# zzbuzzard/PATHS

Measured on AMD Instinct MI355X. Metric: slides_per_sec_5level_K2048_D1024, higher is better.
Workload: dtype f32 (products as 2 fp16 planes per operand = 22 bits, 3 fp16 MFMAs per block, fp32 accumulate); 1 GPU; 5-level PATHS recursion (forward, eval): K=2048 patches/level (level-0 grid 32x64, top_k 512, 10% background), D=1024 features, trans_dim 128 x 4 heads x 2 layers, LSTM ctx 256; 8 HBM-resident slides per GPU; slides_per_gpu=8, global_batch=8, levels=5, resident_batches_rotated=3, parallelism=slide-sharded x1 (no data-path collective)

## Files before the change

### paths_amd/csrc/token0_ws.hip

```cpp
#include "common.h"
#include "lanes.h"

namespace {

constexpr int DM = 128, DFF = 512, NH = 4, HD = 32;
constexpr int NT = 512;
constexpr int SLOTS = NT / 32;
constexpr int REC = 4 + DM;
constexpr int MAX_TS = 16;
constexpr int TS_TOKENS = 128;

constexpr int OFF_A = 0;
constexpr int OFF_A0 = OFF_A + NH * DM * DM;
constexpr int OFF_WV = OFF_A0 + NH * DM;
constexpr int OFF_WO = OFF_WV + DM * DM;
constexpr int OFF_W1 = OFF_WO + DM * DM;
constexpr int OFF_W2 = OFF_W1 + DFF * DM;
constexpr int OFF_OB = OFF_W2 + DM * DFF;
constexpr int IMG_FLOATS = OFF_OB + DM;


struct T0Params {
  const float* x1;
  const int64_t* num_ims;
  const float* img;
  const float *bv, *bo, *ln1g, *ln1b, *cab, *ln2g, *ln2b, *b1, *b2, *ln3g, *ln3b, *lnfg, *lnfb;
  const float* ctx_prev; int64_t ctx_stride; const float* ctx_all; int ctx_depth;
  const float* wcls; const float* bcls; int num_logits, cls_in;
  float* ctx_out; float* logits;
  float* partials;
  int* counters;
  int* status;
  int T, nts; float eps, eps_f;
  int special_last;
};

__device__ __forceinline__ void st_agent(float* p, float v) { __hip_atomic_store(p, v, __ATOMIC_RELAXED, __HIP_MEMORY_SCOPE_AGENT); }
__device__ __forceinline__ float ld_agent(const float* p) { return __hip_atomic_load(p, __ATOMIC_RELAXED, __HIP_MEMORY_SCOPE_AGENT); }
__device__ __forceinline__ float dot4(f32x4 a, f32x4 b) { return fmaf(a[3], b[3], fmaf(a[2], b[2], fmaf(a[1], b[1], a[0] * b[0]))); }

__device__ __forceinline__ void block_layernorm(float* v, const float* g, const float* bta, float eps, int tid) {
  if (tid < 64) {
    const float a = v[tid], c = v[tid + 64];
    const float mean = wave_sum64(a + c) * (1.0f / DM);
    const float da = a - mean, dc = c - mean;
    const float rstd = 1.0f / sqrtf(wave_sum64(da * da + dc * dc) * (1.0f / DM) + eps);
    v[tid] = da * rstd * g[tid] + bta[tid];
    v[tid + 64] = dc * rstd * g[tid + 64] + bta[tid + 64];
  }
  __syncthreads();
}

__global__ void __launch_bounds__(NT)
token0_ws_kernel(T0Params p) {
  __shared__ __attribute__((aligned(16))) float smem[SLOTS * DM + 4 * DFF + 8 * DM + 64];
  float* const sZ = smem;
  float* const sRed = smem + SLOTS * DM;
  float* const sV = sRed + 4 * DFF;
  float* const sX0 = sV, *const sQ = sV + DM, *const sO = sV + 2 * DM, *const sXa = sV + 3 * DM, *const sY = sV + 4 * DM;
  float* const sML = sV + 5 * DM;
  int* const sFlag = reinterpret_cast<int*>(sV + 5 * DM + 2 * SLOTS);
  const int b = blockIdx.y, head = blockIdx.x & 3, ts = blockIdx.x >> 2;
  const int tid = threadIdx.x, lane = tid & 63, wave = tid >> 6;
  const float* xb = p.x1 + (int64_t)b * p.T * DM;

  if (tid < DM) sX0[tid] = xb[(p.special_last ? (int64_t)min((int)p.num_ims[b], p.T - 1) * DM : 0) + tid];
  __syncthreads();
  {
    const int c = tid & 127, kq = tid >> 7;
    const float* A = p.img + OFF_A + (int64_t)head * DM * DM;
    f32x4 w[8];
#pragma unroll
    for (int i = 0; i < 8; ++i) w[i] = ldg_f32x4(A + ((8 * kq + i) * DM + c) * 4);
    float acc = 0.f;
#pragma unroll
    for (int i = 0; i < 8; ++i) acc += dot4(w[i], *reinterpret_cast<const f32x4*>(sX0 + 32 * kq + 4 * i));
    sRed[kq * DM + c] = acc;
  }
  __syncthreads();
  if (tid < DM) sQ[tid] = ((sRed[tid] + sRed[DM + tid]) + (sRed[2 * DM + tid] + sRed[3 * DM + tid])) + p.img[OFF_A0 + head * DM + tid];
  __syncthreads();

  const int len = min((int)p.num_ims[b] + 1, p.T);
  const int chunk = (len + p.nts - 1) / p.nts;
  const int k0 = ts * chunk, k1 = min(len, k0 + chunk);
  const int l5 = lane & 31, slot = wave * 2 + (lane >> 5);
  const f32x4 qv = *reinterpret_cast<const f32x4*>(sQ + 4 * l5);
  float m = -1e30f, l = 0.f;
  f32x4 z = {0.f, 0.f, 0.f, 0.f};
  for (int base = k0; base < k1; base += 8 * SLOTS) {
    f32x4 x[8];
    float s[8];
    bool ok[8];
#pragma unroll
    for (int u = 0; u < 8; ++u) {
      const int tok = base + u * SLOTS + slot;
      ok[u] = tok < k1;
      x[u] = ldg_f32x4(xb + (int64_t)min(tok, k1 - 1) * DM + 4 * l5);
    }
    float mx = m;
#pragma unroll
    for (int u = 0; u < 8; ++u) {
      s[u] = ok[u] ? half_sum32(dot4(qv, x[u])) : -1e30f;
      mx = fmaxf(mx, s[u]);
    }
    const float alpha = __builtin_amdgcn_exp2f(m - mx);
    float ps = 0.f;
    z = z * alpha;
#pragma unroll
    for (int u = 0; u < 8; ++u) {
      const float pu = ok[u] ? __builtin_amdgcn_exp2f(s[u] - mx) : 0.f;
      ps += pu;
      z = z + x[u] * pu;
    }
    l = l * alpha + ps;
    m = mx;
  }
  *reinterpret_cast<f32x4*>(sZ + slot * DM + 4 * l5) = z;
  if (l5 == 0) { sML[2 * slot] = m; sML[2 * slot + 1] = l; }
  __syncthreads();
  float* rec = p.partials + (((int64_t)b * NH + head) * p.nts + ts) * REC;
  if (tid < DM) {
    float M = -1e30f;
#pragma unroll
    for (int sl = 0; sl < SLOTS; ++sl) M = fmaxf(M, sML[2 * sl]);
    float num = 0.f, den = 0.f;
#pragma unroll
    for (int sl = 0; sl < SLOTS; ++sl) {
      const float w = __builtin_amdgcn_exp2f(sML[2 * sl] - M);
      num = fmaf(sZ[sl * DM + tid], w, num);
      den = fmaf(sML[2 * sl + 1], w, den);
    }
    st_agent(rec + 4 + tid, num);
    if (tid == 0) { st_agent(rec, M); st_agent(rec + 1, den); }
  }
  asm volatile("s_waitcnt vmcnt(0)" ::: "memory");
  __syncthreads();
  if (tid == 0) {
    const int total = NH * p.nts;
    const int t = __hip_atomic_fetch_add(p.counters + 3 * b, 1, __ATOMIC_ACQ_REL, __HIP_MEMORY_SCOPE_AGENT);
    const int last = (t == total - 1) ? 1 : 0;
    if (last) {
      __builtin_amdgcn_fence(__ATOMIC_ACQUIRE, "agent");
      __hip_atomic_store(p.counters + 3 * b, 0, __ATOMIC_RELAXED, __HIP_MEMORY_SCOPE_AGENT);
    }
    *sFlag = last;
  }
  __syncthreads();
  if (*sFlag == 0) return;

  const float* W = p.img;
  const int f = tid & 127, kq = tid >> 7;
  float pm[MAX_TS], pl[MAX_TS], pz[MAX_TS];
  {
    const float* hp = p.partials + ((int64_t)b * NH + kq) * p.nts * REC;
#pragma unroll
    for (int t = 0; t < MAX_TS; ++t) {
      const int tc = min(t, p.nts - 1);
      pm[t] = ld_agent(hp + tc * REC); pl[t] = ld_agent(hp + tc * REC + 1); pz[t] = ld_agent(hp + tc * REC + 4 + f);
    }
  }
  f32x4 wv[8], wo[8], w1[32];
#pragma unroll
  for (int i = 0; i < 8; ++i) wv[i] = ldg_f32x4(W + OFF_WV + ((8 * kq + i) * DM + f) * 4);
#pragma unroll
  for (int i = 0; i < 8; ++i) wo[i] = ldg_f32x4(W + OFF_WO + ((8 * kq + i) * DM + f) * 4);
#pragma unroll
  for (int i = 0; i < 32; ++i) w1[i] = ldg_f32x4(W + OFF_W1 + (i * DFF + tid) * 4);
  {
    float M = -1e30f;
#pragma unroll
    for (int t = 0; t < MAX_TS; ++t) if (t < p.nts) M = fmaxf(M, pm[t]);
    float num = 0.f, den = 0.f;
#pragma unroll
    for (int t = 0; t < MAX_TS; ++t)
      if (t < p.nts) {
        const float w = __builtin_amdgcn_exp2f(pm[t] - M);
        num = fmaf(pz[t], w, num);
        den = fmaf(pl[t], w, den);
      }
    sZ[kq * DM + f] = num / den;
  }
  __syncthreads();
  {
    const float* zc = sZ + (f >> 5) * DM + 32 * kq;
    float acc = 0.f;
#pragma unroll
    for (int i = 0; i < 8; ++i) acc += dot4(wv[i], *reinterpret_cast<const f32x4*>(zc + 4 * i));
    sRed[kq * DM + f] = acc;
  }
  __syncthreads();
  if (tid < DM) sO[tid] = ((sRed[tid] + sRed[DM + tid]) + (sRed[2 * DM + tid] + sRed[3 * DM + tid])) + p.bv[tid];
  __syncthreads();
  f32x4 w2[32];
#pragma unroll
  for (int i = 0; i < 16; ++i) w2[i] = ldg_f32x4(W + OFF_W2 + ((32 * kq + i) * DM + f) * 4);
  {
    float acc = 0.f;
#pragma unroll
    for (int i = 0; i < 8; ++i) acc += dot4(wo[i], *reinterpret_cast<const f32x4*>(sO + 32 * kq + 4 * i));
    sRed[kq * DM + f] = acc;
  }
  __syncthreads();
  if (tid < DM) sXa[tid] = sX0[tid] + (((sRed[tid] + sRed[DM + tid]) + (sRed[2 * DM + tid] + sRed[3 * DM + tid])) + p.bo[tid]);
  __syncthreads();
  block_layernorm(sXa, p.ln1g, p.ln1b, p.eps, tid);
  if (tid < DM) sXa[tid] += p.cab[tid];
  __syncthreads();
  block_layernorm(sXa, p.ln2g, p.ln2b, p.eps, tid);
  {
    float acc = 0.f;
#pragma unroll
    for (int i = 0; i < 32; ++i) acc += dot4(w1[i], *reinterpret_cast<const f32x4*>(sXa + 4 * i));
    sRed[tid] = fmaxf(acc + p.b1[tid], 0.f);
  }
#pragma unroll
  for (int i = 16; i < 32; ++i) w2[i] = ldg_f32x4(W + OFF_W2 + ((32 * kq + i) * DM + f) * 4);
  __syncthreads();
  {
    float acc = 0.f;
#pragma unroll
    for (int i = 0; i < 32; ++i) acc += dot4(w2[i], *reinterpret_cast<const f32x4*>(sRed + 128 * kq + 4 * i));
    sZ[kq * DM + f] = acc;
  }
  __syncthreads();
  if (tid < DM) sXa[tid] = sXa[tid] + (((sZ[tid] + sZ[DM + tid]) + (sZ[2 * DM + tid] + sZ[3 * DM + tid])) + p.b2[tid]);
  __syncthreads();
  block_layernorm(sXa, p.ln3g, p.ln3b, p.eps, tid);
  block_layernorm(sXa, p.lnfg, p.lnfb, p.eps_f, tid);
  if (tid < DM) {
    float v = sXa[tid];
    if (p.ctx_prev) v += p.ctx_prev[(int64_t)b * p.ctx_stride + tid];
    sXa[tid] = v;
    p.ctx_out[(int64_t)b * DM + tid] = v;
  }
  __syncthreads();
  for (int j = wave; j < p.num_logits; j += NT / 64) {
    const float* w = p.wcls + (int64_t)j * p.cls_in;
    float acc = 0.f;
    if (p.ctx_all) {
      for (int i = lane; i < p.ctx_depth * DM; i += 64) acc += w[i] * p.ctx_all[(int64_t)b * p.ctx_depth * DM + i];
      w += p.ctx_depth * DM;
    }
    acc += w[lane] * sXa[lane] + w[lane + 64] * sXa[lane + 64];
    acc = wave_sum64(acc);
    if (lane == 0) p.logits[(int64_t)b * p.num_logits + j] = acc + p.bcls[j];
  }
}


constexpr int SPIN_LIMIT = 1 << 22;

template <int D_>
struct T0G {
  static_assert(D_ % 64 == 0 && D_ >= 128 && D_ <= 256, "token0 distributed form: trans_dim 128 or 192 (256 untested)");
  static constexpr int DM = D_, DFF = 4 * D_, HD = D_ / NH, NT = 4 * D_, SLOTS = NT / 32, FPL = D_ / 32, REC = 4 + D_;
  static constexpr int NV = D_ / 64;
  static constexpr int NQ = D_ / 16;
  static constexpr int MAXLD = D_ == 128 ? 8 : D_ / 32;
  static constexpr int RT = D_ == 128 ? 8 : 4;
  static constexpr int OFF_A = 0;
  static constexpr int OFF_A0 = OFF_A + NH * DM * DM;
  static constexpr int OFF_WV = OFF_A0 + NH * DM;
  static constexpr int OFF_WO = OFF_WV + DM * DM;
  static constexpr int OFF_W1 = OFF_WO + DM * DM;
  static constexpr int OFF_W2 = OFF_W1 + DFF * DM;
  static constexpr int OFF_OB = OFF_W2 + DM * DFF;
  static constexpr int IMG_FLOATS = OFF_OB + DM;
  static constexpr int SMEM = SLOTS * DM + 4 * DFF + 8 * DM + 64;
};
static_assert(T0G<128>::OFF_OB == OFF_OB && T0G<128>::IMG_FLOATS == IMG_FLOATS && T0G<128>::REC == REC && T0G<128>::NT == NT, "one image layout at 128");

template <int FPL>
__device__ __forceinline__ void ld_feats(const float* p, float (&x)[FPL]) {
  if constexpr (FPL == 4) {
    const f32x4 t = ldg_f32x4(p);
    x[0] = t[0]; x[1] = t[1]; x[2] = t[2]; x[3] = t[3];
  } else {
    static_assert(FPL % 2 == 0, "features per lane");
    typedef const f32x2 __attribute__((address_space(1))) * gptr;
#pragma unroll
    for (int i = 0; i < FPL / 2; ++i) {
      const f32x2 t = *reinterpret_cast<gptr>(reinterpret_cast<uintptr_t>(p + 2 * i));
      x[2 * i] = t[0]; x[2 * i + 1] = t[1];
    }
  }
}
template <int FPL>
__device__ __forceinline__ float dot_feats(const float (&a)[FPL], const float (&b)[FPL]) {
  float acc = a[0] * b[0];
#pragma unroll
  for (int i = 1; i < FPL; ++i) acc = fmaf(a[i], b[i], acc);
  return acc;
}
template <int D>
__device__ __forceinline__ void block_layernorm_d(float* v, const float* g, const float* bta, float eps, int tid) {
  if (tid < 64) {
    constexpr int VP = D / 64;
    float a[VP], s = 0.f;
#pragma unroll
    for (int i = 0; i < VP; ++i) { a[i] = v[tid + 64 * i]; s += a[i]; }
    const float mean = wave_sum64(s) * (1.0f / D);
    float q = 0.f;
#pragma unroll
    for (int i = 0; i < VP; ++i) { a[i] -= mean; q = fmaf(a[i], a[i], q); }
    const float rstd = 1.0f / sqrtf(wave_sum64(q) * (1.0f / D) + eps);
#pragma unroll
    for (int i = 0; i < VP; ++i) v[tid + 64 * i] = a[i] * rstd * g[tid + 64 * i] + bta[tid + 64 * i];
  }
  __syncthreads();
}

template <int D_>
__global__ void __launch_bounds__(4 * D_)
token0_dist_kernel(T0Params p) {
  using G_ = T0G<D_>;
  constexpr int DM = G_::DM, DFF = G_::DFF, HD = G_::HD, NT = G_::NT, SLOTS = G_::SLOTS, FPL = G_::FPL, REC = G_::REC;
  constexpr int NV = G_::NV, NQ = G_::NQ, MAXLD = G_::MAXLD, RT = G_::RT;
  constexpr int OFF_A = G_::OFF_A, OFF_A0 = G_::OFF_A0, OFF_WV = G_::OFF_WV, OFF_WO = G_::OFF_WO, OFF_W1 = G_::OFF_W1, OFF_W2 = G_::OFF_W2, OFF_OB = G_::OFF_OB;
  __shared__ __attribute__((aligned(16))) float smem[G_::SMEM];
  float* const sZ = smem;
  float* const sRed = smem + SLOTS * DM;
  float* const sV = sRed + 4 * DFF;
  float* const sX0 = sV, *const sQ = sV + DM, *const sNum = sV + 2 * DM, *const sXa = sV + 3 * DM, *const sH = sV + 4 * DM;
  float* const sML = sV + 5 * DM;
  float* const sVv = sV + 5 * DM + 2 * SLOTS + 8;
  int* const sFlag = reinterpret_cast<int*>(sV + 5 * DM + 2 * SLOTS);
  const int G = NH * p.nts, HS = DFF / G, nld = HS / 16;
  const int b = blockIdx.y, j = blockIdx.x, head = j & 3, ts = j >> 2;
  const int tid = threadIdx.x, lane = tid & 63, wave = tid >> 6;
  const float* xb = p.x1 + (int64_t)b * p.T * DM;
  const float* W = p.img;

  const int o5 = tid % HD, kq5 = tid / HD;
  const int f7 = tid % DM, kq7 = tid / DM;
  const int n1 = tid % HS, kq1 = tid / HS;
  f32x4 wv[NV], wo[NV], w1[MAXLD], w2[MAXLD];
#pragma unroll
  for (int i = 0; i < NV; ++i) {
    wv[i] = ldg_f32x4(W + OFF_WV + ((NV * kq5 + i) * DM + HD * head + o5) * 4);
    wo[i] = ldg_f32x4(W + OFF_WO + (((HD / 4) * head + NV * kq7 + i) * DM + f7) * 4);
  }
#pragma unroll
  for (int i = 0; i < MAXLD; ++i)
    if (i < nld) {
      w1[i] = ldg_f32x4(W + OFF_W1 + ((kq1 * nld + i) * DFF + j * HS + n1) * 4);
      w2[i] = ldg_f32x4(W + OFF_W2 + (((j * HS) / 4 + kq7 * nld + i) * DM + f7) * 4);
    }

  constexpr bool A_EARLY = DM == 128;
  const float* const A = W + OFF_A + (int64_t)head * DM * DM;
  f32x4 w[NQ];
  if constexpr (A_EARLY) {
#pragma unroll
    for (int i = 0; i < NQ; ++i) w[i] = ldg_f32x4(A + ((NQ * kq7 + i) * DM + f7) * 4);
  }
  const int len = min((int)p.num_ims[b] + 1, p.T);
  const int chunk = (len + p.nts - 1) / p.nts;
  const int k0 = ts * chunk, k1 = min(len, k0 + chunk);
  const int l5 = lane & 31, slot = wave * 2 + (lane >> 5);
  float xa[RT][FPL], xn[RT][FPL];
  auto fetch = [&](float (&dst)[RT][FPL], int base) __attribute__((always_inline)) {
#pragma unroll
    for (int u = 0; u < RT; ++u) ld_feats<FPL>(xb + (int64_t)max(min(base + u * SLOTS + slot, k1 - 1), 0) * DM + FPL * l5, dst[u]);
  };
  if (A_EARLY && k0 < k1) fetch(xa, k0);

  if (tid < DM) sX0[tid] = xb[(p.special_last ? (int64_t)min((int)p.num_ims[b], p.T - 1) * DM : 0) + tid];
  __syncthreads();
  {
    if constexpr (!A_EARLY) {
#pragma unroll
      for (int i = 0; i < NQ; ++i) w[i] = ldg_f32x4(A + ((NQ * kq7 + i) * DM + f7) * 4);
    }
    float acc = 0.f;
#pragma unroll
    for (int i = 0; i < NQ; ++i) acc += dot4(w[i], *reinterpret_cast<const f32x4*>(sX0 + (DM / 4) * kq7 + 4 * i));
    sRed[kq7 * DM + f7] = acc;
  }
  __syncthreads();
  if (tid < DM) sQ[tid] = ((sRed[tid] + sRed[DM + tid]) + (sRed[2 * DM + tid] + sRed[3 * DM + tid])) + W[OFF_A0 + head * DM + tid];
// ... 44 lines not shown
  if (l5 == 0) { sML[2 * slot] = m; sML[2 * slot + 1] = l; }
  __syncthreads();
  float Mloc = -1e30f;
#pragma unroll
  for (int sl = 0; sl < SLOTS; ++sl) Mloc = fmaxf(Mloc, sML[2 * sl]);
  if (tid < DM) {
    float num = 0.f;
#pragma unroll
    for (int sl = 0; sl < SLOTS; ++sl) num = fmaf(sZ[sl * DM + tid], __builtin_amdgcn_exp2f(sML[2 * sl] - Mloc), num);
    sNum[tid] = num;
  }
  float den = 0.f;
#pragma unroll
  for (int sl = 0; sl < SLOTS; ++sl) den = fmaf(sML[2 * sl + 1], __builtin_amdgcn_exp2f(sML[2 * sl] - Mloc), den);
  __syncthreads();
  {
    float acc = 0.f;
#pragma unroll
    for (int i = 0; i < NV; ++i) acc += dot4(wv[i], *reinterpret_cast<const f32x4*>(sNum + 4 * (NV * kq5 + i)));
    sRed[kq5 * HD + o5] = acc;
  }
  __syncthreads();
  if (tid < HD) {
    float acc = 0.f;
#pragma unroll
    for (int k = 0; k < NT / HD; ++k) acc += sRed[k * HD + tid];
    sVv[tid] = acc;
  }
  __syncthreads();
  {
    float acc = 0.f;
#pragma unroll
    for (int i = 0; i < NV; ++i) acc += dot4(wo[i], *reinterpret_cast<const f32x4*>(sVv + 4 * (NV * kq7 + i)));
    sRed[2 * DFF + kq7 * DM + f7] = acc;
  }
  __syncthreads();
  float* rec = p.partials + ((int64_t)b * G + j) * REC;
  if (tid < DM) {
    const float* r4 = sRed + 2 * DFF + tid;
    st_agent(rec + 4 + tid, (r4[0] + r4[DM]) + (r4[2 * DM] + r4[3 * DM]));
    if (tid == 0) { st_agent(rec, Mloc); st_agent(rec + 1, den); }
  }
  asm volatile("s_waitcnt vmcnt(0)" ::: "memory");
  __syncthreads();
  int* cnt = p.counters + 3 * b;
  if (tid == 0) {
    __hip_atomic_fetch_add(cnt, 1, __ATOMIC_RELEASE, __HIP_MEMORY_SCOPE_AGENT);
    int spins = 0;
    while (__hip_atomic_load(cnt, __ATOMIC_RELAXED, __HIP_MEMORY_SCOPE_AGENT) < G) {
      __builtin_amdgcn_s_sleep(1);
      if (++spins > SPIN_LIMIT) {
        if (p.status) atomicOr(p.status, 4);
        break;
      }
    }
    __builtin_amdgcn_fence(__ATOMIC_ACQUIRE, "agent");
  }
  __syncthreads();
  {
    const int h = kq7;
    const float* hp = p.partials + (int64_t)b * G * REC;
    float pm[8], pl[8], pu[8];
#pragma unroll
    for (int t = 0; t < 8; ++t) {
      const int tc = min(t, p.nts - 1);
      const float* r = hp + (tc * NH + h) * REC;
      pm[t] = ld_agent(r); pl[t] = ld_agent(r + 1); pu[t] = ld_agent(r + 4 + f7);
    }
    float M = -1e30f;
#pragma unroll
    for (int t = 0; t < 8; ++t) if (t < p.nts) M = fmaxf(M, pm[t]);
    float num = 0.f, dn = 0.f;
#pragma unroll
    for (int t = 0; t < 8; ++t)
      if (t < p.nts) {
        const float w = __builtin_amdgcn_exp2f(pm[t] - M);
        num = fmaf(pu[t], w, num);
        dn = fmaf(pl[t], w, dn);
      }
    sRed[h * DM + f7] = num / dn;
  }
  __syncthreads();
  if (tid < DM) sXa[tid] = sX0[tid] + (((sRed[tid] + sRed[DM + tid]) + (sRed[2 * DM + tid] + sRed[3 * DM + tid])) + W[OFF_OB + tid]);
  __syncthreads();
  block_layernorm_d<DM>(sXa, p.ln1g, p.ln1b, p.eps, tid);
  if (tid < DM) sXa[tid] += p.cab[tid];
  __syncthreads();
  block_layernorm_d<DM>(sXa, p.ln2g, p.ln2b, p.eps, tid);
  {
    float acc = 0.f;
#pragma unroll
    for (int i = 0; i < MAXLD; ++i)
      if (i < nld) acc += dot4(w1[i], *reinterpret_cast<const f32x4*>(sXa + (kq1 * nld + i) * 4));
    sRed[kq1 * HS + n1] = acc;
  }
  __syncthreads();
  if (tid < HS) {
    float acc = 0.f;
    const int ng = NT / HS;
    for (int k = 0; k < ng; ++k) acc += sRed[k * HS + tid];
    sH[tid] = fmaxf(acc + p.b1[j * HS + tid], 0.f);
  }
  __syncthreads();
  {
    float acc = 0.f;
#pragma unroll
    for (int i = 0; i < MAXLD; ++i)
      if (i < nld) acc += dot4(w2[i], *reinterpret_cast<const f32x4*>(sH + (kq7 * nld + i) * 4));
    sRed[2 * DFF + kq7 * DM + f7] = acc;
  }
  __syncthreads();
  float* rec2 = p.partials + (int64_t)gridDim.y * (G * REC + DM) + ((int64_t)b * G + j) * DM;
  if (tid < DM) {
    const float* r4 = sRed + 2 * DFF + tid;
    st_agent(rec2 + tid, (r4[0] + r4[DM]) + (r4[2 * DM] + r4[3 * DM]));
  }
  asm volatile("s_waitcnt vmcnt(0)" ::: "memory");
  __syncthreads();
  if (tid == 0) *sFlag = (__hip_atomic_fetch_add(cnt + 2, 1, __ATOMIC_ACQ_REL, __HIP_MEMORY_SCOPE_AGENT) == G - 1) ? 1 : 0;
  __syncthreads();
  if (*sFlag == 0) return;
  if (tid == 0) {
    __hip_atomic_store(cnt, 0, __ATOMIC_RELAXED, __HIP_MEMORY_SCOPE_AGENT);
    __hip_atomic_store(cnt + 2, 0, __ATOMIC_RELAXED, __HIP_MEMORY_SCOPE_AGENT);
  }
  {
    const float* r2 = p.partials + (int64_t)gridDim.y * (G * REC + DM) + (int64_t)b * G * DM;
    float acc = 0.f;
    for (int g = kq7; g < G; g += 4) acc += ld_agent(r2 + g * DM + f7);
    sRed[kq7 * DM + f7] = acc;
  }
  __syncthreads();
  if (tid < DM) sXa[tid] = sXa[tid] + (((sRed[tid] + sRed[DM + tid]) + (sRed[2 * DM + tid] + sRed[3 * DM + tid])) + p.b2[tid]);
  __syncthreads();
  block_layernorm_d<DM>(sXa, p.ln3g, p.ln3b, p.eps, tid);
  block_layernorm_d<DM>(sXa, p.lnfg, p.lnfb, p.eps_f, tid);
  if (tid < DM) {
    float v = sXa[tid];
    if (p.ctx_prev) v += p.ctx_prev[(int64_t)b * p.ctx_stride + tid];
    sXa[tid] = v;
    p.ctx_out[(int64_t)b * DM + tid] = v;
  }
  __syncthreads();
  for (int jj = wave; jj < p.num_logits; jj += NT / 64) {
    const float* w = p.wcls + (int64_t)jj * p.cls_in;
    float acc = 0.f;
    if (p.ctx_all) {
      for (int i = lane; i < p.ctx_depth * DM; i += 64) acc += w[i] * p.ctx_all[(int64_t)b * p.ctx_depth * DM + i];
      w += p.ctx_depth * DM;
    }
#pragma unroll
    for (int i = 0; i < DM / 64; ++i) acc += w[lane + 64 * i] * sXa[lane + 64 * i];
    acc = wave_sum64(acc);
    if (lane == 0) p.logits[(int64_t)b * p.num_logits + jj] = acc + p.bcls[jj];
  }
}

template <int D_>
__global__ void __launch_bounds__(256)
token0_pack_kernel(const float* __restrict__ wqkv, const float* __restrict__ bqkv, const float* __restrict__ wo, const float* __restrict__ bo,
                   const float* __restrict__ w1, const float* __restrict__ w2, float qscale, float* __restrict__ out) {
  using G_ = T0G<D_>;
// ... 4 lines not shown
    if (i >= NH * DM * DM) return;
    const int e = i & 3, c = (i >> 2) % DM, r_ = (i >> 2) / DM, k4 = r_ % (DM / 4), h = r_ / (DM / 4);
    const float* wq = wqkv + (int64_t)(HD * h) * DM + 4 * k4 + e;
    const float* wk = wqkv + (int64_t)(DM + HD * h) * DM + c;
    float acc = 0.f;
    for (int r = 0; r < HD; ++r) acc = fmaf(wk[r * DM], wq[r * DM], acc);
    out[G_::OFF_A + i] = acc * qscale;
  } else if (job == 1) {
    if (i >= NH * DM) return;
    const int c = i % DM, h = i / DM;
    const float* wk = wqkv + (int64_t)(DM + HD * h) * DM + c;
    float acc = 0.f;
    for (int r = 0; r < HD; ++r) acc = fmaf(wk[r * DM], bqkv[HD * h + r], acc);
    out[G_::OFF_A0 + i] = acc * qscale;
  } else if (job == 6) {
    if (i >= DM) return;
    float acc = 0.f;
    for (int k = 0; k < DM; ++k) acc = fmaf(wo[(int64_t)i * DM + k], bqkv[2 * DM + k], acc);
    out[G_::OFF_OB + i] = acc + bo[i];
  } else {
    const float* src; int N, K, off;
    if (job == 2) { src = wqkv + 2 * DM * DM; N = DM; K = DM; off = G_::OFF_WV; }
    else if (job == 3) { src = wo; N = DM; K = DM; off = G_::OFF_WO; }
    else if (job == 4) { src = w1; N = DFF; K = DM; off = G_::OFF_W1; }
    else { src = w2; N = DM; K = DFF; off = G_::OFF_W2; }
    if (i >= N * K) return;
    const int e = i & 3, n = (i >> 2) % N, k4 = (i >> 2) / N;
    out[off + i] = src[(int64_t)n * K + 4 * k4 + e];
  }
}

}

template <int D_>
static int dist_limit() {
  static int cached[64] = {0};
  int dev = 0;
  if (hipGetDevice(&dev) != hipSuccess || dev < 0 || dev >= 64) return 0;
  if (cached[dev] == 0) {
    int cus = 0, occ = 0;
    if (hipDeviceGetAttribute(&cus, hipDeviceAttributeMultiprocessorCount, dev) != hipSuccess || cus <= 0) return 0;
    if (hipOccupancyMaxActiveBlocksPerMultiprocessor(&occ, reinterpret_cast<const void*>(token0_dist_kernel<D_>), T0G<D_>::NT, 0) != hipSuccess || occ <= 0) return 0;
    cached[dev] = cus * (occ > 1 ? 1 : occ) * 3 / 4;
  }
  return cached[dev];
}
static int dist_splits(int B, int T, int d) {
  const int limit = d == 192 ? dist_limit<192>() : dist_limit<128>();
  for (int nts = d == 192 ? 4 : 8; nts >= (d == 192 ? 2 : 1); nts >>= 1)
    if (NH * nts * B <= limit && (nts == 1 || (nts - 1) * TS_TOKENS < T)) return nts;
  return 0;
}
static int chain_splits(int T) {
  int nts = (T + TS_TOKENS - 1) / TS_TOKENS;
  return nts < 1 ? 1 : nts > MAX_TS ? MAX_TS : nts;
}

extern "C" {

int64_t paths_token0_ws_image_bytes_d(int d) { return d == 192 ? (int64_t)T0G<192>::IMG_FLOATS * 4 : d == 128 ? (int64_t)IMG_FLOATS * 4 : 0; }
int64_t paths_token0_ws_image_bytes(void) { return paths_token0_ws_image_bytes_d(128); }

int paths_token0_ws_supported(int B, int T, int d, int H) {
  if (H != NH || B <= 0 || T <= 0) return 0;
  if (d == 128) return 1;
  if (d == 192) return dist_splits(B, T, d) > 0 ? 1 : 0;
  return 0;
}

int64_t paths_token0_ws_partials_d(int B, int T, int d) {
  const int rec = 4 + d;
  const int64_t chain = d == 128 ? (int64_t)B * NH * chain_splits(T) * rec : 0;
  const int nd = dist_splits(B, T, d);
  const int64_t dist = nd ? (int64_t)B * (NH * nd * (rec + d) + d) : 0;
  return chain > dist ? chain : dist;
}
int64_t paths_token0_ws_partials(int B, int T) { return paths_token0_ws_partials_d(B, T, 128); }

int paths_token0_pack_ws_d(const float* wqkv, const float* bqkv, const float* wo, const float* bo, const float* w1, const float* w2, float qscale,
                           int d, void* out, hipStream_t stream) {
  PATHS_REQUIRE(wqkv && bqkv && wo && bo && w1 && w2 && out && (uintptr_t)out % 16 == 0, "token0_pack_ws: bad arguments");
  PATHS_REQUIRE(d == 128 || d == 192, "token0_pack_ws: trans_dim must be 128 or 192 (got %d)", d);
  const dim3 grid((unsigned)(4 * d * d / 256), 7);
  if (d == 192) hipLaunchKernelGGL(token0_pack_kernel<192>, grid, dim3(256), 0, stream, wqkv, bqkv, wo, bo, w1, w2, qscale, reinterpret_cast<float*>(out));
  else hipLaunchKernelGGL(token0_pack_kernel<128>, grid, dim3(256), 0, stream, wqkv, bqkv, wo, bo, w1, w2, qscale, reinterpret_cast<float*>(out));
  PATHS_LAUNCH_CHECK("token0_pack_ws");
  return PATHS_OK;
}
int paths_token0_pack_ws(const float* wqkv, const float* bqkv, const float* wo, const float* bo, const float* w1, const float* w2, float qscale,
                         void* out, hipStream_t stream) {
  return paths_token0_pack_ws_d(wqkv, bqkv, wo, bo, w1, w2, qscale, 128, out, stream);
}

int paths_token0_tail_ws(const float* x1, const int64_t* num_ims, const void* img, const float* bv, const float* bo,
                         const float* ln1g, const float* ln1b, const float* cab, const float* ln2g, const float* ln2b,
                         const float* b1, const float* b2, const float* ln3g, const float* ln3b, const float* lnfg, const float* lnfb,
                         const float* ctx_prev, int64_t ctx_stride, const float* ctx_all, int ctx_depth,
                         const float* wcls, const float* bcls, int num_logits, int cls_in,
                         float* ctx_out, float* logits, float* partials, int* counters, int* status, int B, int T, int d, int H,
                         float eps, float eps_final, int special_last, hipStream_t stream) {
  PATHS_REQUIRE((d == 128 || d == 192) && H == NH, "token0_tail_ws: this build supports trans_dim 128 or 192 with 4 heads (got %d, %d)", d, H);
  PATHS_REQUIRE(B > 0 && T > 0 && x1 && num_ims && img && bv && bo && ln1g && ln1b && cab && ln2g && ln2b && b1 && b2 && ln3g && ln3b && lnfg && lnfb,
                "token0_tail_ws: null operand");
  PATHS_REQUIRE(wcls && bcls && ctx_out && logits && partials && counters, "token0_tail_ws: null output / scratch");
  PATHS_REQUIRE(num_logits > 0 && cls_in == (ctx_all ? (ctx_depth + 1) * d : d), "token0_tail_ws: bad classifier shape");
  PATHS_REQUIRE(((uintptr_t)x1 | (uintptr_t)img) % 16 == 0, "token0_tail_ws: buffers must be 16-byte aligned");
  const int nd = dist_splits(B, T, d);
  if (d != 128 && nd == 0)
    return paths_set_error(PATHS_EUNSUPPORTED, "token0_tail_ws: trans_dim %d has the distributed form only and %d slides do not fit it (paths_token0_ws_supported)", d, B);
  const int nts = nd ? nd : chain_splits(T);
  T0Params p{x1, num_ims, reinterpret_cast<const float*>(img), bv, bo, ln1g, ln1b, cab, ln2g, ln2b, b1, b2, ln3g, ln3b, lnfg, lnfb,
             ctx_prev, ctx_stride, ctx_all, ctx_depth, wcls, bcls, num_logits, cls_in, ctx_out, logits, partials, counters, status, T, nts, eps, eps_final, special_last ? 1 : 0};
  if (nd && d == 192) hipLaunchKernelGGL(token0_dist_kernel<192>, dim3(NH * nts, B), dim3(T0G<192>::NT), 0, stream, p);
  else if (nd) hipLaunchKernelGGL(token0_dist_kernel<128>, dim3(NH * nts, B), dim3(NT), 0, stream, p);
  else hipLaunchKernelGGL(token0_ws_kernel, dim3(NH * nts, B), dim3(NT), 0, stream, p);
  PATHS_LAUNCH_CHECK("token0_tail_ws");
  return PATHS_OK;
}

}
```

Baseline: 3754 slides/s.

## Split token0 tail into pass and chain kernels, replacing grid-wide spin barrier

The distributed token0 kernel used a spin-wait barrier across all attention blocks of a slide before running the feed-forward slices, and a separate chain kernel served other cases. This replaces both with two launches. A pass kernel computes per-head, per-split attention partials. A chain kernel then merges them and computes the FFN across a fixed 8 workgroups per slide, with a last-block reduction. Removing the spin barrier and the occupancy-based split selection avoids co-residency requirements and idle spinning, at the cost of an extra kernel launch and a round trip of the partials through global memory. MAX_TS is lowered to 4.

```diff
diff --git a/paths_amd/csrc/token0_ws.hip b/paths_amd/csrc/token0_ws.hip
--- a/paths_amd/csrc/token0_ws.hip
+++ b/paths_amd/csrc/token0_ws.hip
@@ -3,34 +3,21 @@
 
 namespace {
 
-constexpr int DM = 128, DFF = 512, NH = 4, HD = 32;
-constexpr int NT = 512;
-constexpr int SLOTS = NT / 32;
-constexpr int REC = 4 + DM;
-constexpr int MAX_TS = 16;
+constexpr int NH = 4;
+constexpr int MAX_TS = 4;
 constexpr int TS_TOKENS = 128;
-
-constexpr int OFF_A = 0;
-constexpr int OFF_A0 = OFF_A + NH * DM * DM;
-constexpr int OFF_WV = OFF_A0 + NH * DM;
-constexpr int OFF_WO = OFF_WV + DM * DM;
-constexpr int OFF_W1 = OFF_WO + DM * DM;
-constexpr int OFF_W2 = OFF_W1 + DFF * DM;
-constexpr int OFF_OB = OFF_W2 + DM * DFF;
-constexpr int IMG_FLOATS = OFF_OB + DM;
-
+constexpr int G2 = 8;
 
 struct T0Params {
   const float* x1;
   const int64_t* num_ims;
   const float* img;
-  const float *bv, *bo, *ln1g, *ln1b, *cab, *ln2g, *ln2b, *b1, *b2, *ln3g, *ln3b, *lnfg, *lnfb;
+  const float *ln1g, *ln1b, *cab, *ln2g, *ln2b, *b1, *b2, *ln3g, *ln3b, *lnfg, *lnfb;
   const float* ctx_prev; int64_t ctx_stride; const float* ctx_all; int ctx_depth;
   const float* wcls; const float* bcls; int num_logits, cls_in;
   float* ctx_out; float* logits;
   float* partials;
   int* counters;
-  int* status;
   int T, nts; float eps, eps_f;
   int special_last;
 };
@@ -39,225 +26,15 @@
 __device__ __forceinline__ float ld_agent(const float* p) { return __hip_atomic_load(p, __ATOMIC_RELAXED, __HIP_MEMORY_SCOPE_AGENT); }
 __device__ __forceinline__ float dot4(f32x4 a, f32x4 b) { return fmaf(a[3], b[3], fmaf(a[2], b[2], fmaf(a[1], b[1], a[0] * b[0]))); }
 
-__device__ __forceinline__ void block_layernorm(float* v, const float* g, const float* bta, float eps, int tid) {
-  if (tid < 64) {
-    const float a = v[tid], c = v[tid + 64];
-    const float mean = wave_sum64(a + c) * (1.0f / DM);
-    const float da = a - mean, dc = c - mean;
-    const float rstd = 1.0f / sqrtf(wave_sum64(da * da + dc * dc) * (1.0f / DM) + eps);
-    v[tid] = da * rstd * g[tid] + bta[tid];
-    v[tid + 64] = dc * rstd * g[tid + 64] + bta[tid + 64];
-  }
-  __syncthreads();
-}
-
-__global__ void __launch_bounds__(NT)
-token0_ws_kernel(T0Params p) {
-  __shared__ __attribute__((aligned(16))) float smem[SLOTS * DM + 4 * DFF + 8 * DM + 64];
-  float* const sZ = smem;
-  float* const sRed = smem + SLOTS * DM;
-  float* const sV = sRed + 4 * DFF;
-  float* const sX0 = sV, *const sQ = sV + DM, *const sO = sV + 2 * DM, *const sXa = sV + 3 * DM, *const sY = sV + 4 * DM;
-  float* const sML = sV + 5 * DM;
-  int* const sFlag = reinterpret_cast<int*>(sV + 5 * DM + 2 * SLOTS);
-  const int b = blockIdx.y, head = blockIdx.x & 3, ts = blockIdx.x >> 2;
-  const int tid = threadIdx.x, lane = tid & 63, wave = tid >> 6;
-  const float* xb = p.x1 + (int64_t)b * p.T * DM;
-
-  if (tid < DM) sX0[tid] = xb[(p.special_last ? (int64_t)min((int)p.num_ims[b], p.T - 1) * DM : 0) + tid];
-  __syncthreads();
-  {
-    const int c = tid & 127, kq = tid >> 7;
-    const float* A = p.img + OFF_A + (int64_t)head * DM * DM;
-    f32x4 w[8];
-#pragma unroll
-    for (int i = 0; i < 8; ++i) w[i] = ldg_f32x4(A + ((8 * kq + i) * DM + c) * 4);
-    float acc = 0.f;
-#pragma unroll
-    for (int i = 0; i < 8; ++i) acc += dot4(w[i], *reinterpret_cast<const f32x4*>(sX0 + 32 * kq + 4 * i));
-    sRed[kq * DM + c] = acc;
-  }
-  __syncthreads();
-  if (tid < DM) sQ[tid] = ((sRed[tid] + sRed[DM + tid]) + (sRed[2 * DM + tid] + sRed[3 * DM + tid])) + p.img[OFF_A0 + head * DM + tid];
-  __syncthreads();
-
-  const int len = min((int)p.num_ims[b] + 1, p.T);
-  const int chunk = (len + p.nts - 1) / p.nts;
-  const int k0 = ts * chunk, k1 = min(len, k0 + chunk);
-  const int l5 = lane & 31, slot = wave * 2 + (lane >> 5);
-  const f32x4 qv = *reinterpret_cast<const f32x4*>(sQ + 4 * l5);
-  float m = -1e30f, l = 0.f;
-  f32x4 z = {0.f, 0.f, 0.f, 0.f};
-  for (int base = k0; base < k1; base += 8 * SLOTS) {
-    f32x4 x[8];
-    float s[8];
-    bool ok[8];
-#pragma unroll
-    for (int u = 0; u < 8; ++u) {
-      const int tok = base + u * SLOTS + slot;
-      ok[u] = tok < k1;
-      x[u] = ldg_f32x4(xb + (int64_t)min(tok, k1 - 1) * DM + 4 * l5);
-    }
-    float mx = m;
-#pragma unroll
-    for (int u = 0; u < 8; ++u) {
-      s[u] = ok[u] ? half_sum32(dot4(qv, x[u])) : -1e30f;
-      mx = fmaxf(mx, s[u]);
-    }
-    const float alpha = __builtin_amdgcn_exp2f(m - mx);
-    float ps = 0.f;
-    z = z * alpha;
-#pragma unroll
-    for (int u = 0; u < 8; ++u) {
-      const float pu = ok[u] ? __builtin_amdgcn_exp2f(s[u] - mx) : 0.f;
-      ps += pu;
-      z = z + x[u] * pu;
-    }
-    l = l * alpha + ps;
-    m = mx;
-  }
-  *reinterpret_cast<f32x4*>(sZ + slot * DM + 4 * l5) = z;
-  if (l5 == 0) { sML[2 * slot] = m; sML[2 * slot + 1] = l; }
-  __syncthreads();
-  float* rec = p.partials + (((int64_t)b * NH + head) * p.nts + ts) * REC;
-  if (tid < DM) {
-    float M = -1e30f;
-#pragma unroll
-    for (int sl = 0; sl < SLOTS; ++sl) M = fmaxf(M, sML[2 * sl]);
-    float num = 0.f, den = 0.f;
-#pragma unroll
-    for (int sl = 0; sl < SLOTS; ++sl) {
-      const float w = __builtin_amdgcn_exp2f(sML[2 * sl] - M);
-      num = fmaf(sZ[sl * DM + tid], w, num);
-      den = fmaf(sML[2 * sl + 1], w, den);
-    }
-    st_agent(rec + 4 + tid, num);
-    if (tid == 0) { st_agent(rec, M); st_agent(rec + 1, den); }
-  }
-  asm volatile("s_waitcnt vmcnt(0)" ::: "memory");
-  __syncthreads();
-  if (tid == 0) {
-    const int total = NH * p.nts;
-    const int t = __hip_atomic_fetch_add(p.counters + 3 * b, 1, __ATOMIC_ACQ_REL, __HIP_MEMORY_SCOPE_AGENT);
-    const int last = (t == total - 1) ? 1 : 0;
-    if (last) {
-      __builtin_amdgcn_fence(__ATOMIC_ACQUIRE, "agent");
-      __hip_atomic_store(p.counters + 3 * b, 0, __ATOMIC_RELAXED, __HIP_MEMORY_SCOPE_AGENT);
-    }
-    *sFlag = last;
-  }
-  __syncthreads();
-  if (*sFlag == 0) return;
-
-  const float* W = p.img;
-  const int f = tid & 127, kq = tid >> 7;
-  float pm[MAX_TS], pl[MAX_TS], pz[MAX_TS];
-  {
-    const float* hp = p.partials + ((int64_t)b * NH + kq) * p.nts * REC;
-#pragma unroll
-    for (int t = 0; t < MAX_TS; ++t) {
-      const int tc = min(t, p.nts - 1);
-      pm[t] = ld_agent(hp + tc * REC); pl[t] = ld_agent(hp + tc * REC + 1); pz[t] = ld_agent(hp + tc * REC + 4 + f);
-    }
-  }
-  f32x4 wv[8], wo[8], w1[32];
-#pragma unroll
-  for (int i = 0; i < 8; ++i) wv[i] = ldg_f32x4(W + OFF_WV + ((8 * kq + i) * DM + f) * 4);
-#pragma unroll
-  for (int i = 0; i < 8; ++i) wo[i] = ldg_f32x4(W + OFF_WO + ((8 * kq + i) * DM + f) * 4);
-#pragma unroll
-  for (int i = 0; i < 32; ++i) w1[i] = ldg_f32x4(W + OFF_W1 + (i * DFF + tid) * 4);
-  {
-    float M = -1e30f;
-#pragma unroll
-    for (int t = 0; t < MAX_TS; ++t) if (t < p.nts) M = fmaxf(M, pm[t]);
-    float num = 0.f, den = 0.f;
-#pragma unroll
-    for (int t = 0; t < MAX_TS; ++t)
-      if (t < p.nts) {
-        const float w = __builtin_amdgcn_exp2f(pm[t] - M);
-        num = fmaf(pz[t], w, num);
-        den = fmaf(pl[t], w, den);
-      }
-    sZ[kq * DM + f] = num / den;
-  }
-  __syncthreads();
-  {
-    const float* zc = sZ + (f >> 5) * DM + 32 * kq;
-    float acc = 0.f;
-#pragma unroll
-    for (int i = 0; i < 8; ++i) acc += dot4(wv[i], *reinterpret_cast<const f32x4*>(zc + 4 * i));
-    sRed[kq * DM + f] = acc;
-  }
-  __syncthreads();
-  if (tid < DM) sO[tid] = ((sRed[tid] + sRed[DM + tid]) + (sRed[2 * DM + tid] + sRed[3 * DM + tid])) + p.bv[tid];
-  __syncthreads();
-  f32x4 w2[32];
-#pragma unroll
-  for (int i = 0; i < 16; ++i) w2[i] = ldg_f32x4(W + OFF_W2 + ((32 * kq + i) * DM + f) * 4);
-  {
-    float acc = 0.f;
-#pragma unroll
-    for (int i = 0; i < 8; ++i) acc += dot4(wo[i], *reinterpret_cast<const f32x4*>(sO + 32 * kq + 4 * i));
-    sRed[kq * DM + f] = acc;
-  }
-  __syncthreads();
-  if (tid < DM) sXa[tid] = sX0[tid] + (((sRed[tid] + sRed[DM + tid]) + (sRed[2 * DM + tid] + sRed[3 * DM + tid])) + p.bo[tid]);
-  __syncthreads();
-  block_layernorm(sXa, p.ln1g, p.ln1b, p.eps, tid);
-  if (tid < DM) sXa[tid] += p.cab[tid];
-  __syncthreads();
-  block_layernorm(sXa, p.ln2g, p.ln2b, p.eps, tid);
-  {
-    float acc = 0.f;
-#pragma unroll
-    for (int i = 0; i < 32; ++i) acc += dot4(w1[i], *reinterpret_cast<const f32x4*>(sXa + 4 * i));
-    sRed[tid] = fmaxf(acc + p.b1[tid], 0.f);
-  }
-#pragma unroll
-  for (int i = 16; i < 32; ++i) w2[i] = ldg_f32x4(W + OFF_W2 + ((32 * kq + i) * DM + f) * 4);
-  __syncthreads();
-  {
-    float acc = 0.f;
-#pragma unroll
-    for (int i = 0; i < 32; ++i) acc += dot4(w2[i], *reinterpret_cast<const f32x4*>(sRed + 128 * kq + 4 * i));
-    sZ[kq * DM + f] = acc;
-  }
-  __syncthreads();
-  if (tid < DM) sXa[tid] = sXa[tid] + (((sZ[tid] + sZ[DM + tid]) + (sZ[2 * DM + tid] + sZ[3 * DM + tid])) + p.b2[tid]);
-  __syncthreads();
-  block_layernorm(sXa, p.ln3g, p.ln3b, p.eps, tid);
-  block_layernorm(sXa, p.lnfg, p.lnfb, p.eps_f, tid);
-  if (tid < DM) {
-    float v = sXa[tid];
-    if (p.ctx_prev) v += p.ctx_prev[(int64_t)b * p.ctx_stride + tid];
-    sXa[tid] = v;
-    p.ctx_out[(int64_t)b * DM + tid] = v;
-  }
-  __syncthreads();
-  for (int j = wave; j < p.num_logits; j += NT / 64) {
-    const float* w = p.wcls + (int64_t)j * p.cls_in;
-    float acc = 0.f;
-    if (p.ctx_all) {
-      for (int i = lane; i < p.ctx_depth * DM; i += 64) acc += w[i] * p.ctx_all[(int64_t)b * p.ctx_depth * DM + i];
-      w += p.ctx_depth * DM;
-    }
-    acc += w[lane] * sXa[lane] + w[lane + 64] * sXa[lane + 64];
-    acc = wave_sum64(acc);
-    if (lane == 0) p.logits[(int64_t)b * p.num_logits + j] = acc + p.bcls[j];
-  }
-}
-
-
-constexpr int SPIN_LIMIT = 1 << 22;
-
 template <int D_>
 struct T0G {
-  static_assert(D_ % 64 == 0 && D_ >= 128 && D_ <= 256, "token0 distributed form: trans_dim 128 or 192 (256 untested)");
+  static_assert(D_ % 64 == 0 && D_ >= 128 && D_ <= 256, "token0 tail: trans_dim 128 or 192 (256 untested)");
   static constexpr int DM = D_, DFF = 4 * D_, HD = D_ / NH, NT = 4 * D_, SLOTS = NT / 32, FPL = D_ / 32, REC = 4 + D_;
   static constexpr int NV = D_ / 64;
   static constexpr int NQ = D_ / 16;
-  static constexpr int MAXLD = D_ == 128 ? 8 : D_ / 32;
+  static constexpr int HS = 4 * D_ / G2;
+  static constexpr int NLD = HS / 16;
+  static_assert(HS % 16 == 0 && (4 * D_) % HS == 0 && HS <= D_, "feed-forward slice: a multiple of 16 hidden units that divides the workgroup");
   static constexpr int RT = D_ == 128 ? 8 : 4;
   static constexpr int OFF_A = 0;
   static constexpr int OFF_A0 = OFF_A + NH * DM * DM;
@@ -267,9 +44,9 @@
   static constexpr int OFF_W2 = OFF_W1 + DFF * DM;
   static constexpr int OFF_OB = OFF_W2 + DM * DFF;
   static constexpr int IMG_FLOATS = OFF_OB + DM;
-  static constexpr int SMEM = SLOTS * DM + 4 * DFF + 8 * DM + 64;
+  static constexpr int SMEM_PASS = SLOTS * DM + 8 * DM + 4 * DM + 2 * SLOTS + 8 + HD;
+  static constexpr int SMEM_CHAIN = 8 * DM + 3 * DM + 8;
 };
-static_assert(T0G<128>::OFF_OB == OFF_OB && T0G<128>::IMG_FLOATS == IMG_FLOATS && T0G<128>::REC == REC && T0G<128>::NT == NT, "one image layout at 128");
 
 template <int FPL>
 __device__ __forceinline__ void ld_feats(const float* p, float (&x)[FPL]) {
@@ -313,20 +90,19 @@
 
 template <int D_>
 __global__ void __launch_bounds__(4 * D_)
-token0_dist_kernel(T0Params p) {
+token0_pass_kernel(T0Params p) {
   using G_ = T0G<D_>;
-  constexpr int DM = G_::DM, DFF = G_::DFF, HD = G_::HD, NT = G_::NT, SLOTS = G_::SLOTS, FPL = G_::FPL, REC = G_::REC;
-  constexpr int NV = G_::NV, NQ = G_::NQ, MAXLD = G_::MAXLD, RT = G_::RT;
-  constexpr int OFF_A = G_::OFF_A, OFF_A0 = G_::OFF_A0, OFF_WV = G_::OFF_WV, OFF_WO = G_::OFF_WO, OFF_W1 = G_::OFF_W1, OFF_W2 = G_::OFF_W2, OFF_OB = G_::OFF_OB;
-  __shared__ __attribute__((aligned(16))) float smem[G_::SMEM];
+  constexpr int DM = G_::DM, HD = G_::HD, NT = G_::NT, SLOTS = G_::SLOTS, FPL = G_::FPL, REC = G_::REC;
+  constexpr int NV = G_::NV, NQ = G_::NQ, RT = G_::RT;
+  constexpr int OFF_A = G_::OFF_A, OFF_A0 = G_::OFF_A0, OFF_WV = G_::OFF_WV, OFF_WO = G_::OFF_WO;
+  __shared__ __attribute__((aligned(16))) float smem[G_::SMEM_PASS];
   float* const sZ = smem;
   float* const sRed = smem + SLOTS * DM;
-  float* const sV = sRed + 4 * DFF;
-  float* const sX0 = sV, *const sQ = sV + DM, *const sNum = sV + 2 * DM, *const sXa = sV + 3 * DM, *const sH = sV + 4 * DM;
-  float* const sML = sV + 5 * DM;
-  float* const sVv = sV + 5 * DM + 2 * SLOTS + 8;
-  int* const sFlag = reinterpret_cast<int*>(sV + 5 * DM + 2 * SLOTS);
-  const int G = NH * p.nts, HS = DFF / G, nld = HS / 16;
+  float* const sRed2 = sRed + 4 * DM;
+  float* const sV = sRed + 8 * DM;
+  float* const sX0 = sV, *const sQ = sV + DM, *const sNum = sV + 2 * DM;
+  float* const sML = sV + 4 * DM;
+  float* const sVv = sV + 4 * DM + 2 * SLOTS + 8;
   const int b = blockIdx.y, j = blockIdx.x, head = j & 3, ts = j >> 2;
   const int tid = threadIdx.x, lane = tid & 63, wave = tid >> 6;
   const float* xb = p.x1 + (int64_t)b * p.T * DM;
@@ -334,19 +110,12 @@
 
   const int o5 = tid % HD, kq5 = tid / HD;
   const int f7 = tid % DM, kq7 = tid / DM;
-  const int n1 = tid % HS, kq1 = tid / HS;
-  f32x4 wv[NV], wo[NV], w1[MAXLD], w2[MAXLD];
+  f32x4 wv[NV], wo[NV];
 #pragma unroll
   for (int i = 0; i < NV; ++i) {
     wv[i] = ldg_f32x4(W + OFF_WV + ((NV * kq5 + i) * DM + HD * head + o5) * 4);
     wo[i] = ldg_f32x4(W + OFF_WO + (((HD / 4) * head + NV * kq7 + i) * DM + f7) * 4);
   }
-#pragma unroll
-  for (int i = 0; i < MAXLD; ++i)
-    if (i < nld) {
-      w1[i] = ldg_f32x4(W + OFF_W1 + ((kq1 * nld + i) * DFF + j * HS + n1) * 4);
-      w2[i] = ldg_f32x4(W + OFF_W2 + (((j * HS) / 4 + kq7 * nld + i) * DM + f7) * 4);
-    }
 
   constexpr bool A_EARLY = DM == 128;
   const float* const A = W + OFF_A + (int64_t)head * DM * DM;
@@ -457,52 +226,55 @@
     float acc = 0.f;
 #pragma unroll
     for (int i = 0; i < NV; ++i) acc += dot4(wo[i], *reinterpret_cast<const f32x4*>(sVv + 4 * (NV * kq7 + i)));
-    sRed[2 * DFF + kq7 * DM + f7] = acc;
-  }
-  __syncthreads();
-  float* rec = p.partials + ((int64_t)b * G + j) * REC;
+    sRed2[kq7 * DM + f7] = acc;
+  }
+  __syncthreads();
+  float* rec = p.partials + ((int64_t)b * NH * p.nts + j) * REC;
   if (tid < DM) {
-    const float* r4 = sRed + 2 * DFF + tid;
-    st_agent(rec + 4 + tid, (r4[0] + r4[DM]) + (r4[2 * DM] + r4[3 * DM]));
-    if (tid == 0) { st_agent(rec, Mloc); st_agent(rec + 1, den); }
-  }
-  asm volatile("s_waitcnt vmcnt(0)" ::: "memory");
-  __syncthreads();
-  int* cnt = p.counters + 3 * b;
-  if (tid == 0) {
-    __hip_atomic_fetch_add(cnt, 1, __ATOMIC_RELEASE, __HIP_MEMORY_SCOPE_AGENT);
-    int spins = 0;
-    while (__hip_atomic_load(cnt, __ATOMIC_RELAXED, __HIP_MEMORY_SCOPE_AGENT) < G) {
-      __builtin_amdgcn_s_sleep(1);
-      if (++spins > SPIN_LIMIT) {
-        if (p.status) atomicOr(p.status, 4);
-        break;
-      }
-    }
-    __builtin_amdgcn_fence(__ATOMIC_ACQUIRE, "agent");
-  }
-  __syncthreads();
+    const float* r4 = sRed2 + tid;
+    rec[4 + tid] = (r4[0] + r4[DM]) + (r4[2 * DM] + r4[3 * DM]);
+    if (tid == 0) { rec[0] = Mloc; rec[1] = den; }
+  }
+}
+
+template <int D_>
+__global__ void __launch_bounds__(4 * D_)
+token0_chain_kernel(T0Params p) {
+  using G_ = T0G<D_>;
+  constexpr int DM = G_::DM, DFF = G_::DFF, NT = G_::NT, REC = G_::REC, HS = G_::HS, NLD = G_::NLD;
+  constexpr int OFF_W1 = G_::OFF_W1, OFF_W2 = G_::OFF_W2, OFF_OB = G_::OFF_OB;
+  __shared__ __attribute__((aligned(16))) float smem[G_::SMEM_CHAIN];
+  float* const sRed = smem;
+  float* const sRed2 = smem + 4 * DM;
+  float* const sX0 = smem + 8 * DM, *const sXa = sX0 + DM, *const sH = sX0 + 2 * DM;
+  int* const sFlag = reinterpret_cast<int*>(sX0 + 3 * DM);
+  const int b = blockIdx.y, j = blockIdx.x;
+  const int tid = threadIdx.x, lane = tid & 63, wave = tid >> 6;
+  const float* xb = p.x1 + (int64_t)b * p.T * DM;
+  const float* W = p.img;
+
+  const int f7 = tid % DM, kq7 = tid / DM;
+  const int n1 = tid % HS, kq1 = tid / HS;
+  f32x4 w1[NLD], w2[NLD];
+#pragma unroll
+  for (int i = 0; i < NLD; ++i) {
+    w1[i] = ldg_f32x4(W + OFF_W1 + ((kq1 * NLD + i) * DFF + j * HS + n1) * 4);
+    w2[i] = ldg_f32x4(W + OFF_W2 + (((j * HS) / 4 + kq7 * NLD + i) * DM + f7) * 4);
+  }
+  if (tid < DM) sX0[tid] = xb[(p.special_last ? (int64_t)min((int)p.num_ims[b], p.T - 1) * DM : 0) + tid];
   {
     const int h = kq7;
-    const float* hp = p.partials + (int64_t)b * G * REC;
-    float pm[8], pl[8], pu[8];
-#pragma unroll
-    for (int t = 0; t < 8; ++t) {
-      const int tc = min(t, p.nts - 1);
-      const float* r = hp + (tc * NH + h) * REC;
-      pm[t] = ld_agent(r); pl[t] = ld_agent(r + 1); pu[t] = ld_agent(r + 4 + f7);
-    }
+    const float* hp = p.partials + ((int64_t)b * NH * p.nts + h) * REC;
     float M = -1e30f;
-#pragma unroll
-    for (int t = 0; t < 8; ++t) if (t < p.nts) M = fmaxf(M, pm[t]);
+    for (int t = 0; t < p.nts; ++t) M = fmaxf(M, hp[t * NH * REC]);
     float num = 0.f, dn = 0.f;
-#pragma unroll
-    for (int t = 0; t < 8; ++t)
-      if (t < p.nts) {
-        const float w = __builtin_amdgcn_exp2f(pm[t] - M);
-        num = fmaf(pu[t], w, num);
-        dn = fmaf(pl[t], w, dn);
-      }
+#pragma unroll 4
+    for (int t = 0; t < p.nts; ++t) {
+      const float* r = hp + t * NH * REC;
+      const float w = __builtin_amdgcn_exp2f(r[0] - M);
+      num = fmaf(r[4 + f7], w, num);
+      dn = fmaf(r[1], w, dn);
+    }
     sRed[h * DM + f7] = num / dn;
   }
   __syncthreads();
@@ -515,44 +287,46 @@
   {
     float acc = 0.f;
 #pragma unroll
-    for (int i = 0; i < MAXLD; ++i)
-      if (i < nld) acc += dot4(w1[i], *reinterpret_cast<const f32x4*>(sXa + (kq1 * nld + i) * 4));
+    for (int i = 0; i < NLD; ++i) acc += dot4(w1[i], *reinterpret_cast<const f32x4*>(sXa + (kq1 * NLD + i) * 4));
     sRed[kq1 * HS + n1] = acc;
   }
   __syncthreads();
   if (tid < HS) {
     float acc = 0.f;
-    const int ng = NT / HS;
-    for (int k = 0; k < ng; ++k) acc += sRed[k * HS + tid];
+    for (int k = 0; k < NT / HS; ++k) acc += sRed[k * HS + tid];
     sH[tid] = fmaxf(acc + p.b1[j * HS + tid], 0.f);
   }
   __syncthreads();
   {
     float acc = 0.f;
 #pragma unroll
-    for (int i = 0; i < MAXLD; ++i)
-      if (i < nld) acc += dot4(w2[i], *reinterpret_cast<const f32x4*>(sH + (kq7 * nld + i) * 4));
-    sRed[2 * DFF + kq7 * DM + f7] = acc;
-  }
-  __syncthreads();
-  float* rec2 = p.partials + (int64_t)gridDim.y * (G * REC + DM) + ((int64_t)b * G + j) * DM;
+    for (int i = 0; i < NLD; ++i) acc += dot4(w2[i], *reinterpret_cast<const f32x4*>(sH + (kq7 * NLD + i) * 4));
+    sRed2[kq7 * DM + f7] = acc;
+  }
+  __syncthreads();
+  float* const ybase = p.partials + (int64_t)gridDim.y * NH * p.nts * REC + (int64_t)b * G2 * DM;
+  float* rec2 = ybase + j * DM;
   if (tid < DM) {
-    const float* r4 = sRed + 2 * DFF + tid;
+    const float* r4 = sRed2 + tid;
     st_agent(rec2 + tid, (r4[0] + r4[DM]) + (r4[2 * DM] + r4[3 * DM]));
   }
   asm volatile("s_waitcnt vmcnt(0)" ::: "memory");
   __syncthreads();
-  if (tid == 0) *sFlag = (__hip_atomic_fetch_add(cnt + 2, 1, __ATOMIC_ACQ_REL, __HIP_MEMORY_SCOPE_AGENT) == G - 1) ? 1 : 0;
+  int* cnt = p.counters + 3 * b + 2;
+  if (tid == 0) {
+    const int last = (__hip_atomic_fetch_add(cnt, 1, __ATOMIC_ACQ_REL, __HIP_MEMORY_SCOPE_AGENT) == G2 - 1) ? 1 : 0;
+    if (last) {
+      __builtin_amdgcn_fence(__ATOMIC_ACQUIRE, "agent");
+      __hip_atomic_store(cnt, 0, __ATOMIC_RELAXED, __HIP_MEMORY_SCOPE_AGENT);
+    }
+    *sFlag = last;
+  }
   __syncthreads();
   if (*sFlag == 0) return;
-  if (tid == 0) {
-    __hip_atomic_store(cnt, 0, __ATOMIC_RELAXED, __HIP_MEMORY_SCOPE_AGENT);
-    __hip_atomic_store(cnt + 2, 0, __ATOMIC_RELAXED, __HIP_MEMORY_SCOPE_AGENT);
-  }
-  {
-    const float* r2 = p.partials + (int64_t)gridDim.y * (G * REC + DM) + (int64_t)b * G * DM;
-    float acc = 0.f;
-    for (int g = kq7; g < G; g += 4) acc += ld_agent(r2 + g * DM + f7);
+  {
+    const float* r2 = ybase;
+    float acc = 0.f;
+    for (int g = kq7; g < G2; g += 4) acc += ld_agent(r2 + g * DM + f7);
     sRed[kq7 * DM + f7] = acc;
   }
   __syncthreads();
@@ -623,48 +397,25 @@
 
 }
 
-template <int D_>
-static int dist_limit() {
-  static int cached[64] = {0};
-  int dev = 0;
-  if (hipGetDevice(&dev) != hipSuccess || dev < 0 || dev >= 64) return 0;
-  if (cached[dev] == 0) {
-    int cus = 0, occ = 0;
-    if (hipDeviceGetAttribute(&cus, hipDeviceAttributeMultiprocessorCount, dev) != hipSuccess || cus <= 0) return 0;
-    if (hipOccupancyMaxActiveBlocksPerMultiprocessor(&occ, reinterpret_cast<const void*>(token0_dist_kernel<D_>), T0G<D_>::NT, 0) != hipSuccess || occ <= 0) return 0;
-    cached[dev] = cus * (occ > 1 ? 1 : occ) * 3 / 4;
-  }
-  return cached[dev];
-}
-static int dist_splits(int B, int T, int d) {
-  const int limit = d == 192 ? dist_limit<192>() : dist_limit<128>();
-  for (int nts = d == 192 ? 4 : 8; nts >= (d == 192 ? 2 : 1); nts >>= 1)
-    if (NH * nts * B <= limit && (nts == 1 || (nts - 1) * TS_TOKENS < T)) return nts;
-  return 0;
-}
-static int chain_splits(int T) {
-  int nts = (T + TS_TOKENS - 1) / TS_TOKENS;
+static int pass_splits(int T) {
+  const int nts = (T + TS_TOKENS - 1) / TS_TOKENS;
   return nts < 1 ? 1 : nts > MAX_TS ? MAX_TS : nts;
 }
 
 extern "C" {
 
-int64_t paths_token0_ws_image_bytes_d(int d) { return d == 192 ? (int64_t)T0G<192>::IMG_FLOATS * 4 : d == 128 ? (int64_t)IMG_FLOATS * 4 : 0; }
+int64_t paths_token0_ws_image_bytes_d(int d) { return d == 192 ? (int64_t)T0G<192>::IMG_FLOATS * 4 : d == 128 ? (int64_t)T0G<128>::IMG_FLOATS * 4 : 0; }
 int64_t paths_token0_ws_image_bytes(void) { return paths_token0_ws_image_bytes_d(128); }
 
 int paths_token0_ws_supported(int B, int T, int d, int H) {
   if (H != NH || B <= 0 || T <= 0) return 0;
   if (d == 128) return 1;
-  if (d == 192) return dist_splits(B, T, d) > 0 ? 1 : 0;
+  if (d == 192) return T > TS_TOKENS ? 1 : 0;
   return 0;
 }
 
 int64_t paths_token0_ws_partials_d(int B, int T, int d) {
-  const int rec = 4 + d;
-  const int64_t chain = d == 128 ? (int64_t)B * NH * chain_splits(T) * rec : 0;
-  const int nd = dist_splits(B, T, d);
-  const int64_t dist = nd ? (int64_t)B * (NH * nd * (rec + d) + d) : 0;
-  return chain > dist ? chain : dist;
+  return (int64_t)B * (NH * pass_splits(T) * (4 + d) + G2 * d);
 }
 int64_t paths_token0_ws_partials(int B, int T) { return paths_token0_ws_partials_d(B, T, 128); }
 
@@ -696,15 +447,19 @@
   PATHS_REQUIRE(wcls && bcls && ctx_out && logits && partials && counters, "token0_tail_ws: null output / scratch");
   PATHS_REQUIRE(num_logits > 0 && cls_in == (ctx_all ? (ctx_depth + 1) * d : d), "token0_tail_ws: bad classifier shape");
   PATHS_REQUIRE(((uintptr_t)x1 | (uintptr_t)img) % 16 == 0, "token0_tail_ws: buffers must be 16-byte aligned");
-  const int nd = dist_splits(B, T, d);
-  if (d != 128 && nd == 0)
-    return paths_set_error(PATHS_EUNSUPPORTED, "token0_tail_ws: trans_dim %d has the distributed form only and %d slides do not fit it (paths_token0_ws_supported)", d, B);
-  const int nts = nd ? nd : chain_splits(T);
-  T0Params p{x1, num_ims, reinterpret_cast<const float*>(img), bv, bo, ln1g, ln1b, cab, ln2g, ln2b, b1, b2, ln3g, ln3b, lnfg, lnfb,
-             ctx_prev, ctx_stride, ctx_all, ctx_depth, wcls, bcls, num_logits, cls_in, ctx_out, logits, partials, counters, status, T, nts, eps, eps_final, special_last ? 1 : 0};
-  if (nd && d == 192) hipLaunchKernelGGL(token0_dist_kernel<192>, dim3(NH * nts, B), dim3(T0G<192>::NT), 0, stream, p);
-  else if (nd) hipLaunchKernelGGL(token0_dist_kernel<128>, dim3(NH * nts, B), dim3(NT), 0, stream, p);
-  else hipLaunchKernelGGL(token0_ws_kernel, dim3(NH * nts, B), dim3(NT), 0, stream, p);
+  if (!paths_token0_ws_supported(B, T, d, H))
+    return paths_set_error(PATHS_EUNSUPPORTED, "token0_tail_ws: trans_dim %d needs T > %d (got %d; paths_token0_ws_supported)", d, TS_TOKENS, T);
+  (void)status;
+  const int nts = pass_splits(T);
+  T0Params p{x1, num_ims, reinterpret_cast<const float*>(img), ln1g, ln1b, cab, ln2g, ln2b, b1, b2, ln3g, ln3b, lnfg, lnfb,
+             ctx_prev, ctx_stride, ctx_all, ctx_depth, wcls, bcls, num_logits, cls_in, ctx_out, logits, partials, counters, T, nts, eps, eps_final, special_last ? 1 : 0};
+  if (d == 192) {
+    hipLaunchKernelGGL(token0_pass_kernel<192>, dim3(NH * nts, B), dim3(T0G<192>::NT), 0, stream, p);
+    hipLaunchKernelGGL(token0_chain_kernel<192>, dim3(G2, B), dim3(T0G<192>::NT), 0, stream, p);
+  } else {
+    hipLaunchKernelGGL(token0_pass_kernel<128>, dim3(NH * nts, B), dim3(T0G<128>::NT), 0, stream, p);
+    hipLaunchKernelGGL(token0_chain_kernel<128>, dim3(G2, B), dim3(T0G<128>::NT), 0, stream, p);
+  }
   PATHS_LAUNCH_CHECK("token0_tail_ws");
   return PATHS_OK;
 }
```

After: 3768 slides/s, median of 6. About the same (+0.4%).
